# tonyzyl/ladcast

Measured on AMD Instinct MI355X. Metric: ensemble-member-steps/sec, higher is better.
Workload: dtype f32

## Files before the change

### include/ladcast_hip.h

```cpp
#ifndef LADCAST_HIP_H
#define LADCAST_HIP_H

#ifdef __cplusplus
extern "C" {
#endif

#define LDC_ABI_VERSION 5

#define LDC_OK 0
#define LDC_ERR_ARG (-1)
#define LDC_ERR_ALIGN (-2)
#define LDC_ERR_UNSUPPORTED (-3)

enum ldc_act { LDC_ACT_NONE = 0, LDC_ACT_SILU = 1, LDC_ACT_GELU_TANH = 2, LDC_ACT_RELU = 3 };
#define LDC_ACT_IN_TIMESTEP_SINCOS 16

int ldc_abi_version(void);
const char* ldc_build_arch(void);

typedef struct ldc_gemm_desc {
  int M, N, K, batch;
  int lda, ldw, ldc, ldr;
  long long a_bs, c_bs, r_bs;
  int gate_bs;
  int act;
  int flags;
  int reserved;
} ldc_gemm_desc;
#define LDC_GEMM_A_SPLIT 1
#define LDC_GEMM_C_SPLIT 2
#define LDC_GEMM_BF16_1TERM 4
#define LDC_GEMM_F32_REGSTAGE 8
#define LDC_FMT_F32 0
#define LDC_FMT_SPLIT 1
#define LDC_FMT_BF16 2
int ldc_sizeof_gemm_desc(void);
int ldc_gemm_bias_act(const float* A, const float* W, const float* bias, const float* gate,
                      const float* R, float* C, const ldc_gemm_desc* d, void* stream);

#define LDC_GEMM_MAX_PROBLEMS 4
typedef struct ldc_gemm_problem {
  const float* A;
  const float* W;
  const float* bias;
  const float* gate;
  const float* R;
  float* C;
  ldc_gemm_desc d;
} ldc_gemm_problem;
int ldc_sizeof_gemm_problem(void);
long long ldc_gemm_grouped_workspace_bytes(void);
int ldc_gemm_grouped_workspace_init(void* workspace, long long workspace_bytes, void* stream);
int ldc_gemm_grouped(const ldc_gemm_problem* problems, int n, void* workspace, long long workspace_bytes,
                     void* stream);

int ldc_gemm_grouped_bf16x3(const ldc_gemm_problem* problems, int n, void* workspace, long long workspace_bytes,
                            void* stream);
int ldc_pack_weight_bf16x2(const float* W, void* out, int N, int K, int ldw, void* stream);
int ldc_pack_weight_bf16(const float* W, void* out, int N, int K, int ldw, void* stream);

int ldc_linear_small(const float* x, int x_rows, const float* W, const float* bias,
                     const float* add, int add_rows, float* y, int rows, int N, int K,
                     int act_in, int act_out, void* stream);

int ldc_linear_small_mod(const float* x, int x_rows, const float* W, const float* bias, const float* add, int add_rows,
                         const float* mod, int mod_rows, float* y, int rows, int N, int K, int act_in, int act_out,
                         void* stream);

#define LDC_LINEAR_SMALL_MAX_GROUPED 4
typedef struct ldc_linear_small_problem {
  const float* x;
  const float* W;
  const float* bias;
  const float* add;
  float* y;
  int x_rows, add_rows, rows, N, K, act_in, act_out, reserved;
} ldc_linear_small_problem;
int ldc_linear_small_grouped(const ldc_linear_small_problem* problems, int n, void* stream);

int ldc_attn_fwd(const float* Q, const float* K, const float* V, float* O, int B, int S, int H,
                 int ld_qkv, long long qkv_bs, int ldo, long long o_bs, const float* key_bias, void* stream);
long long ldc_attn_fwd_workspace_bytes(void);
int ldc_attn_fwd_ws(const float* Q, const float* K, const float* V, float* O, int B, int S, int H, int ld_qkv, long long qkv_bs,
                    int ldo, long long o_bs, const float* key_bias, void* workspace, long long workspace_bytes, void* stream);
int ldc_attn_fwd_qrows(const float* Q, const float* K, const float* V, float* O, int B, int S, int Sq, int H, int ld_qkv,
                       long long qkv_bs, int ldo, long long o_bs, const float* key_bias, void* stream);
int ldc_attn_fwd_ws_qrows(const float* Q, const float* K, const float* V, float* O, int B, int S, int Sq, int H, int ld_qkv,
// ... 237 lines not shown
```

### ladcast_amd/csrc/gemm_bf16x3_v3.hip

```cpp
#include <math.h>
#include <stdio.h>
#include <stdlib.h>

#include "common.h"

namespace {

#include "gemm_v3_common.inc"
#include "gemm_v3_kstep_f32.inc"

struct SKArgs {
  DevProblem pr[MAXP];
  int np;
  int G;
  long long U;
  long long tiles;
  float* ws;
  unsigned* counters;
  unsigned upg, urem;
};

__device__ __forceinline__ long long range_start(long long g, const SKArgs& a) {
  const unsigned gu = static_cast<unsigned>(g);
  return static_cast<long long>(gu * a.upg + (gu < a.urem ? gu : a.urem));
}

__device__ __forceinline__ int find_problem_by_unit(const SKArgs& a, long long u) {
  int pi = 0;
#pragma unroll
  for (int k = 1; k < MAXP; ++k)
    if (k < a.np && u >= a.pr[k].unit0) pi = k;
  return pi;
}

#ifdef LDC_GEMM_STAMPS
#define LDC_STAMP(i)                                                                                        \
  if (threadIdx.x == 0)                                                                                     \
    reinterpret_cast<unsigned long long*>(a.counters)[65536 + blockIdx.x * 16 + (i)] = __builtin_amdgcn_s_memrealtime();
#define LDC_STAMP_CLK(i)                                                                                    \
  if (threadIdx.x == 0)                                                                                     \
    reinterpret_cast<unsigned long long*>(a.counters)[65536 + blockIdx.x * 16 + (i)] = __builtin_amdgcn_s_memtime();
#else
#define LDC_STAMP(i)
#define LDC_STAMP_CLK(i)
#endif

template <int BM, int TERMS, bool CONV = false>
__global__ __launch_bounds__(512) void gemm_bf16x3_v3_kernel(SKArgs a) {
  constexpr int CPK = TERMS == 1 ? 2 * BK : BK;
  constexpr int RT = BM / 128;
  constexpr int NACC = RT * 8;
  constexpr int STAGE_B = (BM + BN) * ROW_B;
  constexpr int SLOT_FLOATS = BM * BN;
  constexpr int NAI = BM / 64;
  constexpr int ND = NAI + 2;
  constexpr int NDH = ND / 2;
  extern __shared__ __attribute__((aligned(16))) unsigned char smem[];
  const int wave = __builtin_amdgcn_readfirstlane(static_cast<int>(threadIdx.x) >> 6);
  LDC_STAMP(0)
  int seg_ = 0;
  (void)seg_;
  int g;
  {
    const int bid = blockIdx.x, G = a.G;
    const int q = G >> 3, r = G & 7, xcd = bid & 7;
    g = (xcd < r ? xcd * (q + 1) : r * (q + 1) + (xcd - r) * q) + (bid >> 3);
  }
  auto uniform64 = [](long long v) {
    const unsigned lo = __builtin_amdgcn_readfirstlane(static_cast<unsigned>(v));
    const unsigned hi = __builtin_amdgcn_readfirstlane(static_cast<unsigned>(static_cast<unsigned long long>(v) >> 32));
    return static_cast<long long>((static_cast<unsigned long long>(hi) << 32) | lo);
  };
  const long long u_begin = uniform64(range_start(g, a));
  const long long u_end = uniform64(range_start(g + 1, a));
  const unsigned smem_lds = lds_addr(smem);

  struct Seg {
    int pi, tile, k0, k1, b, bm, bn;
  };
  auto decode = [&](long long u_) {
    Seg sg;
    sg.pi = find_problem_by_unit(a, u_);
    const DevProblem& Q = a.pr[sg.pi];
    const unsigned local = static_cast<unsigned>(u_ - Q.unit0), kt_u = static_cast<unsigned>(Q.kt);
    sg.tile = __builtin_amdgcn_readfirstlane(static_cast<int>(local / kt_u));
    sg.k0 = static_cast<int>(local - static_cast<unsigned>(sg.tile) * kt_u);
    const long long left = u_end - u_;
    sg.k1 = (Q.kt - sg.k0 <= left) ? Q.kt : sg.k0 + static_cast<int>(left);
    const unsigned per_b = static_cast<unsigned>(Q.tm * Q.tn), tile_u = static_cast<unsigned>(sg.tile);
    const unsigned b_ = tile_u / per_b;
    const unsigned t_in = tile_u - b_ * per_b;
    const unsigned strip = static_cast<unsigned>(Q.rm * Q.tn);
    const unsigned sr = t_in / strip;
    const unsigned r_in = t_in - sr * strip;
    const int rest = Q.tm - static_cast<int>(sr) * Q.rm;
    const unsigned h_sr = static_cast<unsigned>(rest < Q.rm ? rest : Q.rm);
    const unsigned bn_ = r_in / h_sr;
    sg.b = __builtin_amdgcn_readfirstlane(static_cast<int>(b_));
    sg.bn = __builtin_amdgcn_readfirstlane(static_cast<int>(bn_));
    sg.bm = __builtin_amdgcn_readfirstlane(static_cast<int>(sr) * Q.rm + static_cast<int>(r_in - bn_ * h_sr));
    return sg;
  };
  auto prefetch_next = [&](const Seg& sg) __attribute__((always_inline)) {
    const DevProblem& Q = a.pr[sg.pi];
    const int ln = fresh_lane();
    const int lr_ = ln >> 3, lp_ = ln & 7;
    const float* __restrict__ An = Q.A + static_cast<long long>(sg.b) * Q.d.a_bs;
    const long long wrb = static_cast<long long>(Q.d.K) * (TERMS == 1 ? 2 : 4);
    unsigned char* dump = smem + NSTAGE * STAGE_B + wave * 1024;
#pragma unroll
    for (int j = 0; j < 2; ++j) {
      const bool live = sg.k0 + j < sg.k1;
      const long long koff = static_cast<long long>(live ? sg.k0 + j : sg.k1 - 1) * (BK * 4);
      unsigned char* sA = smem + j * STAGE_B;
      unsigned char* sW = sA + BM * ROW_B;
#pragma unroll
      for (int i = 0; i < NAI; ++i) {
        const int r = 8 * (wave + 8 * i) + lr_;
        int gm = sg.bm * BM + r;
        gm = gm < Q.d.M ? gm : Q.d.M - 1;
        dma16(reinterpret_cast<const unsigned char*>(An + static_cast<long long>(gm) * Q.d.lda) + ((lp_ ^ swz(r)) << 4) + koff,
              live ? sA + (wave + 8 * i) * 1024 : dump);
      }
#pragma unroll
      for (int i = 0; i < 2; ++i) {
        const int r = 8 * (wave + 8 * i) + lr_;
        int gn = sg.bn * BN + r;
        gn = gn < Q.d.N ? gn : Q.d.N - 1;
        dma16(Q.W + static_cast<long long>(gn) * wrb + ((lp_ ^ swz(r)) << 4) + koff, live ? sW + (wave + 8 * (i)) * 1024 : dump);
      }
    }
  };
  long long u = u_begin;
// ... 304 lines not shown
#undef LDC_MMF
#undef LDC_MM
#undef LDC_RD_A
#undef LDC_RD_W
#undef LDC_SB
    __builtin_amdgcn_s_barrier();
    prefetched = false;
    if constexpr (!CONV && TERMS == 0) {
#if !defined(LDC_GEMM_DIAG_NODMA) && !defined(LDC_GEMM_NO_PREFETCH)
      if (u_next < u_end) {
        prefetch_next(nxt);
        prefetched = true;
      }
#endif
    }
    if (seg_ == 0) { LDC_STAMP_CLK(14) }
    LDC_STAMP(2 + 4 * seg_)

    if (k0 == 0 && k1 == P.kt) {
      tile_epilogue<BM, !CONV, LinearRows<BM>, true, TERMS == 0>(P, b, bm, bn, acc, wave, lane);
    } else {
      const int lane_h = fresh_lane();
      float* slot = a.ws + (static_cast<long long>(2 * g) + (k0 > 0 ? 0 : 1)) * SLOT_FLOATS + lane_h;
#pragma unroll
      for (int i = 0; i < NACC; ++i)
#pragma unroll
        for (int r = 0; r < 4; ++r)
          __hip_atomic_store(slot + ((wave * NACC + i) * 4 + r) * 64, acc[i][r], __ATOMIC_RELAXED, __HIP_MEMORY_SCOPE_AGENT);
      asm volatile("s_waitcnt vmcnt(0)" ::: "memory");
      __builtin_amdgcn_s_barrier();
      const long long f = P.unit0 + static_cast<long long>(tile) * P.kt;
      const long long l = f + P.kt;
      long long g_first = g;
      while (g_first > 0 && range_start(g_first, a) > f) --g_first;
      long long g_last = g;
      while (g_last + 1 < a.G && range_start(g_last + 1, a) < l) ++g_last;
      const unsigned pieces = static_cast<unsigned>(g_last - g_first + 1);
      unsigned* cnt = a.counters + (P.tile0 + tile);
      unsigned* flag = reinterpret_cast<unsigned*>(smem + NSTAGE * STAGE_B);
      if (wave == 0 && lane_h == 0) {
        const unsigned ticket = __hip_atomic_fetch_add(cnt, 1u, __ATOMIC_RELAXED, __HIP_MEMORY_SCOPE_AGENT);
        const unsigned last = (ticket == pieces - 1) ? 1u : 0u;
        if (last) {
          __builtin_amdgcn_fence(__ATOMIC_ACQUIRE, "agent");
          asm volatile("s_waitcnt vmcnt(0)" ::: "memory");
          __hip_atomic_store(cnt, 0u, __ATOMIC_RELAXED, __HIP_MEMORY_SCOPE_AGENT);
        }
        *flag = last;
      }
      __syncthreads();
      LDC_STAMP(3 + 4 * seg_)
      const unsigned is_last = *flag;
      __syncthreads();
      if (is_last) {
#pragma unroll
        for (int i = 0; i < NACC; ++i) acc[i] = f32x4{0.f, 0.f, 0.f, 0.f};
        for (long long gp = g_first; gp <= g_last; ++gp) {
          const long long s = range_start(gp, a);
          const float* sl = a.ws + (2 * gp + (s > f ? 0 : 1)) * SLOT_FLOATS;
#pragma unroll
          for (int i = 0; i < NACC; ++i) {
#pragma unroll
            for (int r = 0; r < 4; ++r) acc[i][r] += sl[((wave * NACC + i) * 4 + r) * 64 + lane_h];
          }
        }
        tile_epilogue<BM, !CONV, LinearRows<BM>, true, TERMS == 0>(P, b, bm, bn, acc, wave, lane);
      }
    }
    u = u_next;
    cur = nxt;
    LDC_STAMP(4 + 4 * seg_)
#ifdef LDC_GEMM_STAMPS
    if (seg_ < 2) ++seg_;
#endif
  }
  LDC_STAMP(15)
}

struct ConvParams {
  int H, W, cin, ks, kshift;
};

constexpr int LDC_SPLIT_GROUP = -100;

template <int BM, int TERMS, bool CONV = false>
int launch_v3(const ldc_gemm_problem* problems, const ldc_qkv_epilogue* epi, int n, void* workspace, long long workspace_bytes,
              void* stream, const ConvParams* cp = nullptr, bool may_split_group = false) {
  constexpr int SLOT_FLOATS = BM * BN;
  constexpr int STAGE_B = (BM + BN) * ROW_B;
  constexpr int CUS = 256;
  SKArgs a{};
  a.np = n;
  long long U = 0, tiles = 0;
  for (int i = 0; i < n; ++i) {
    const ldc_gemm_problem& q = problems[i];
    LDC_CHECK_PTR(q.A);
    LDC_CHECK_PTR(q.W);
    LDC_CHECK_PTR(q.C);
    const ldc_gemm_desc& d = q.d;
    if (d.M <= 0 || d.N <= 0 || d.K <= 0 || d.batch <= 0) return LDC_ERR_ARG;
    if (d.K % (TERMS == 1 ? 2 * BK : BK)) return LDC_ERR_UNSUPPORTED;
    if constexpr (TERMS == 0) {
      if (d.flags != 0 || d.ldw != d.K) return LDC_ERR_UNSUPPORTED;
    } else {
      if (!(d.flags & LDC_GEMM_A_SPLIT)) return LDC_ERR_UNSUPPORTED;
    }
    LDC_CHECK_ALIGN16(q.A);
    LDC_CHECK_ALIGN16(q.W);
    if constexpr (TERMS == 0) {
      if ((d.lda & 3) || (d.a_bs & 3)) return LDC_ERR_UNSUPPORTED;
    } else {
      if ((d.lda & 7) || (d.a_bs & 7) || (reinterpret_cast<unsigned long long>(q.A) & 31ull)) return LDC_ERR_ALIGN;
    }
    if (d.act < LDC_ACT_NONE || d.act > LDC_ACT_RELU) return LDC_ERR_UNSUPPORTED;
    DevProblem& P = a.pr[i];
    P.A = q.A;
    P.W = reinterpret_cast<const unsigned char*>(q.W);
    P.bias = q.bias;
    P.gate = q.gate;
    P.R = q.R;
// ... 105 lines not shown
  }
  if constexpr (TERMS == 0) {
    if (U >= 4 * CUS) G = CUS;
  }
  static const char* const force_g = LDC_AB_GETENV("LDC_BF16X3_G");
  if (force_g) {
    const long long g_ = atoll(force_g);
    if (g_ > 0 && g_ <= CUS) G = g_;
  }
  if (U < G) G = U;
  if (workspace == nullptr) return LDC_ERR_ARG;
  if (workspace_bytes < LDC_GEMM_COUNTER_BYTES + 2 * slot_bytes) return LDC_ERR_ARG;
  {
    const long long fit = (workspace_bytes - LDC_GEMM_COUNTER_BYTES) / (2 * slot_bytes);
    if (fit < G) G = fit;
  }
  LDC_CHECK_ALIGN16(workspace);
  if (U >= (1LL << 31)) return LDC_ERR_UNSUPPORTED;
#ifdef LDC_AB_BUILD
  {
    static const bool dbg = getenv("LDC_GEMM_DEBUG_G") != nullptr;
    if (dbg)
      fprintf(stderr, "ldc_gemm cut: terms %d conv %d n %d tiles %lld kt0 %d BM %d G %lld U %lld %s\n", TERMS, int(CONV), n, tiles, a.pr[0].kt, BM, G, U,
              (U % G == 0 && (U / G) % a.pr[0].kt == 0) ? "whole tiles" : (U % G == 0 ? "equal ranges" : "UNALIGNED"));
  }
#endif
  a.G = static_cast<int>(G);
  a.U = U;
  a.upg = static_cast<unsigned>(U / G);
  a.urem = static_cast<unsigned>(U % G);
  a.tiles = tiles;
  a.ws = reinterpret_cast<float*>(static_cast<unsigned char*>(workspace) + LDC_GEMM_COUNTER_BYTES);
  a.counters = static_cast<unsigned*>(workspace);
  const size_t lds = NSTAGE * STAGE_B + 8 * 1024;
  static const bool attr_set = [&] {
    (void)hipFuncSetAttribute(reinterpret_cast<const void*>(gemm_bf16x3_v3_kernel<BM, TERMS, CONV>),
                              hipFuncAttributeMaxDynamicSharedMemorySize, static_cast<int>(lds));
    return true;
  }();
  (void)attr_set;
  hipLaunchKernelGGL((gemm_bf16x3_v3_kernel<BM, TERMS, CONV>), dim3(a.G), dim3(512), lds, static_cast<hipStream_t>(stream), a);
  return ldc_launch_status();
}

}

static int gemm_v3_dispatch(const ldc_gemm_problem* problems, const ldc_qkv_epilogue* epi, int n, void* workspace,
                            long long workspace_bytes, void* stream) {
  LDC_CHECK_PTR(problems);
  if (n <= 0 || n > MAXP) return LDC_ERR_ARG;
  long long tiles256 = 0;
  for (int i = 0; i < n; ++i) {
    const ldc_gemm_desc& d = problems[i].d;
    if (d.M <= 0 || d.N <= 0 || d.batch <= 0) return LDC_ERR_ARG;
    if (!(d.flags & LDC_GEMM_A_SPLIT)) return LDC_ERR_UNSUPPORTED;
    if (((d.flags ^ problems[0].d.flags) & LDC_GEMM_BF16_1TERM) != 0) return LDC_ERR_ARG;
    tiles256 += static_cast<long long>(d.batch) * ldc_cdiv(d.M, 256) * ldc_cdiv(d.N, BN);
  }
  static const char* const force_thr = LDC_AB_GETENV("LDC_BF16X3_SMALL_TILES");
  bool small = tiles256 < (force_thr ? atoll(force_thr) : 400);
  static const char* const force_bm = LDC_AB_GETENV("LDC_BF16X3_BM");
  if (force_bm) small = (atoi(force_bm) == 128);
  const bool one = (problems[0].d.flags & LDC_GEMM_BF16_1TERM) != 0;
  auto launch = [&](const ldc_gemm_problem* pr, const ldc_qkv_epilogue* ep, int cnt, bool sm, bool may_split) {
    if (one)
      return sm ? launch_v3<128, 1>(pr, ep, cnt, workspace, workspace_bytes, stream, nullptr, may_split)
                : launch_v3<256, 1>(pr, ep, cnt, workspace, workspace_bytes, stream, nullptr, may_split);
    return sm ? launch_v3<128, 3>(pr, ep, cnt, workspace, workspace_bytes, stream, nullptr, may_split)
              : launch_v3<256, 3>(pr, ep, cnt, workspace, workspace_bytes, stream, nullptr, may_split);
  };
  const int st = launch(problems, epi, n, small, true);
  if (st != LDC_SPLIT_GROUP) return st;
  for (int i = 0; i < n; ++i) {
    const ldc_gemm_desc& d = problems[i].d;
    bool sm = static_cast<long long>(d.batch) * ldc_cdiv(d.M, 256) * ldc_cdiv(d.N, BN) < (force_thr ? atoll(force_thr) : 400);
    if (force_bm) sm = (atoi(force_bm) == 128);
    const int sti = launch(problems + i, epi ? epi + i : nullptr, 1, sm, false);
    if (sti != LDC_OK) return sti;
  }
  return LDC_OK;
}

static int gemm_f32_ring(const ldc_gemm_problem* problems, const ldc_qkv_epilogue* epi, int n, void* workspace, long long workspace_bytes,
                         void* stream) {
  LDC_CHECK_PTR(problems);
  if (n <= 0 || n > MAXP) return LDC_ERR_ARG;
  for (int i = 0; i < n; ++i)
    if (problems[i].d.flags & LDC_GEMM_F32_REGSTAGE) return LDC_ERR_UNSUPPORTED;
  auto al16 = [](const void* q_) { return q_ != nullptr && (reinterpret_cast<unsigned long long>(q_) & 15ull) == 0; };
  if (!al16(workspace) || workspace_bytes < LDC_GEMM_COUNTER_BYTES + 2ll * 256 * BN * static_cast<long long>(sizeof(float)))
    return LDC_ERR_UNSUPPORTED;
  for (int i = 0; i < n; ++i) {
    const ldc_gemm_desc& d = problems[i].d;
    if (d.M <= 0 || d.N <= 0 || d.K <= 0 || d.batch <= 0) return LDC_ERR_ARG;
    if (!al16(problems[i].A) || !al16(problems[i].W)) return LDC_ERR_UNSUPPORTED;
  }
#ifdef LDC_AB_BUILD
  static const char* const force_bm = getenv("LDC_F32_RING_BM");
  if (force_bm && atoi(force_bm) == 256) return launch_v3<256, 0>(problems, epi, n, workspace, workspace_bytes, stream);
#endif
  return launch_v3<128, 0>(problems, epi, n, workspace, workspace_bytes, stream);
}

int ldc_gemm_grouped_f32_ring(const ldc_gemm_problem* problems, int n, void* workspace, long long workspace_bytes, void* stream) {
  return gemm_f32_ring(problems, nullptr, n, workspace, workspace_bytes, stream);
}

extern "C" int ldc_gemm_grouped_qkv_f32(const ldc_gemm_problem* problems, const ldc_qkv_epilogue* epi, int n, void* workspace,
                                        long long workspace_bytes, void* stream) {
  LDC_CHECK_PTR(epi);
  return gemm_f32_ring(problems, epi, n, workspace, workspace_bytes, stream);
}

int ldc_gemm_grouped_bf16x3_v3(const ldc_gemm_problem* problems, int n, void* workspace, long long workspace_bytes,
                               void* stream) {
  return gemm_v3_dispatch(problems, nullptr, n, workspace, workspace_bytes, stream);
}

extern "C" int ldc_gemm_grouped_bf16x3_qkv(const ldc_gemm_problem* problems, const ldc_qkv_epilogue* epi, int n, void* workspace,
                                           long long workspace_bytes, void* stream) {
  LDC_CHECK_PTR(epi);
  return gemm_v3_dispatch(problems, epi, n, workspace, workspace_bytes, stream);
}

extern "C" int ldc_sphere_conv_nhwc_split(const float* X, const void* Wp, const float* bias, const float* R, float* Y, int B, int H,
                                          int W, int cin, int ldx, int cout, int ldy, int ldr, int ksize, int act, int in_fmt,
                                          int out_fmt, void* workspace, long long workspace_bytes, void* stream) {
  LDC_CHECK_PTR(X);
  LDC_CHECK_PTR(Wp);
  LDC_CHECK_PTR(Y);
  if (B <= 0 || H <= 0 || W <= 0 || cin <= 0 || cout <= 0) return LDC_ERR_ARG;
  if (ksize != 1 && ksize != 3 && ksize != 5) return LDC_ERR_UNSUPPORTED;
  if (ksize > 1 && ((W & 1) || H < 2 || H < ksize / 2 || W / 2 < ksize / 2 || H > 32767 || W > 65535)) return LDC_ERR_UNSUPPORTED;
  if (in_fmt != LDC_FMT_SPLIT && in_fmt != LDC_FMT_BF16 && in_fmt != LDC_FMT_F32) return LDC_ERR_UNSUPPORTED;
// ... 52 lines not shown
```

### ladcast_amd/hip.py

```python
from __future__ import annotations

import ctypes
import os
from ctypes import POINTER, Structure, c_char_p, c_double, c_float, c_int, c_longlong, c_void_p

import torch

_HERE = os.path.dirname(os.path.abspath(__file__))
LIB_PATH = os.environ.get("LDC_LIB_PATH") or os.path.join(_HERE, "libladcast_hip.so")

ACT_NONE, ACT_SILU, ACT_GELU_TANH, ACT_RELU = 0, 1, 2, 3
ACT_IN_TIMESTEP_SINCOS = 16
GEMM_A_SPLIT, GEMM_C_SPLIT, GEMM_BF16_1TERM = 1, 2, 4
GEMM_F32_REGSTAGE = 8
ATTN_OUT_SPLIT, ATTN_BF16_1TERM, ATTN_OUT_BF16 = 1, 2, 4
ABI_VERSION = 5
FMT_F32, FMT_SPLIT, FMT_BF16 = 0, 1, 2


class GemmDesc(Structure):
    _fields_ = [
        ("M", c_int), ("N", c_int), ("K", c_int), ("batch", c_int),
        ("lda", c_int), ("ldw", c_int), ("ldc", c_int), ("ldr", c_int),
        ("a_bs", c_longlong), ("c_bs", c_longlong), ("r_bs", c_longlong),
        ("gate_bs", c_int), ("act", c_int), ("flags", c_int), ("reserved", c_int),
    ]


class GemmProblem(Structure):
    _fields_ = [("A", c_void_p), ("W", c_void_p), ("bias", c_void_p), ("gate", c_void_p), ("R", c_void_p), ("C", c_void_p), ("d", GemmDesc)]


MAX_GROUPED = 4


class QkvEpilogue(Structure):
    _fields_ = [("wq", c_void_p), ("wk", c_void_p), ("rope", c_void_p), ("reserved", c_void_p), ("eps", c_float), ("qscale", c_float),
                ("heads", c_int), ("rope_row0", c_int)]


class LinearSmallProblem(Structure):
    _fields_ = [("x", c_void_p), ("W", c_void_p), ("bias", c_void_p), ("add", c_void_p), ("y", c_void_p), ("x_rows", c_int), ("add_rows", c_int),
                ("rows", c_int), ("N", c_int), ("K", c_int), ("act_in", c_int), ("act_out", c_int), ("reserved", c_int)]


PRODUCTS_MAX_QUANTILES, PRODUCTS_MAX_THRESHOLDS, PRODUCTS_MAX_MEMBERS, PRODUCTS_MAX_SORT_MEMBERS = 16, 8, 1024, 64


class ProductsDesc(Structure):
    _fields_ = [("n_quant", c_int), ("n_thr", c_int), ("q_lo", c_int * PRODUCTS_MAX_QUANTILES), ("q_t", c_float * PRODUCTS_MAX_QUANTILES),
                ("thr_dir", c_int * PRODUCTS_MAX_THRESHOLDS)]


EVENTS_MAX, EVENTS_MAX_MEMBERS = 32, 1024


class EventsDesc(Structure):
    _fields_ = [("n_events", c_int), ("channel", c_int * EVENTS_MAX), ("dir", c_int * EVENTS_MAX), ("anomaly", c_int * EVENTS_MAX),
                ("thr", c_float * EVENTS_MAX)]


def _load():
    if not os.path.exists(LIB_PATH):
        raise RuntimeError(
            f"{LIB_PATH} is missing: build it with `python -c 'import __graft_entry__ as g; g.build()'` "
            "(or `make -C ladcast_amd/csrc`).  ladcast_amd has no CPU fallback."
        )
    lib = ctypes.CDLL(LIB_PATH)
    P, I, L, F, D = c_void_p, c_int, c_longlong, c_float, c_double
    sig = {
        "ldc_abi_version": (I, []),
        "ldc_build_arch": (c_char_p, []),
        "ldc_sizeof_gemm_desc": (I, []),
        "ldc_gemm_bias_act": (I, [P, P, P, P, P, P, POINTER(GemmDesc), P]),
        "ldc_sizeof_gemm_problem": (I, []),
        "ldc_gemm_grouped_workspace_bytes": (L, []),
        "ldc_gemm_grouped_workspace_init": (I, [P, L, P]),
        "ldc_gemm_grouped": (I, [POINTER(GemmProblem), I, P, L, P]),
        "ldc_gemm_grouped_bf16x3": (I, [POINTER(GemmProblem), I, P, L, P]),
        "ldc_sizeof_qkv_epilogue": (I, []),
        "ldc_gemm_grouped_bf16x3_qkv": (I, [POINTER(GemmProblem), POINTER(QkvEpilogue), I, P, L, P]),
        "ldc_gemm_grouped_qkv_f32": (I, [POINTER(GemmProblem), POINTER(QkvEpilogue), I, P, L, P]),
        "ldc_attn_qkv_prepare_split": (I, [P, P, P, I, I, I, I, L, I, P, P, P, P, P, P, P, P, F, P]),
        "ldc_attn_fwd_split_workspace_bytes": (L, [I, I, I]),
        "ldc_attn_fwd_split_workspace_max_bytes": (L, []),
        "ldc_attn_fwd_split": (I, [P, P, P, P, I, I, I, I, L, I, L, P, I, P, L, P]),
        "ldc_attn_fwd_split_qrows_workspace_bytes": (L, [I, I, I, I]),
        "ldc_attn_fwd_split_qrows": (I, [P, P, P, P, I, I, I, I, I, L, I, L, P, I, P, L, P]),
        "ldc_pack_weight_bf16x2": (I, [P, P, I, I, I, P]),
        "ldc_pack_weight_bf16": (I, [P, P, I, I, I, P]),
        "ldc_linear_small": (I, [P, I, P, P, P, I, P, I, I, I, I, I, P]),
        "ldc_linear_small_grouped": (I, [POINTER(LinearSmallProblem), I, P]),
        "ldc_linear_small_mod": (I, [P, I, P, P, P, I, P, I, P, I, I, I, I, I, P]),
        "ldc_gate_residual_layernorm": (I, [P, P, P, P, I, I, I, I, L, I, L, I, I, L, P, P, F, I, P]),
        "ldc_attn_fwd": (I, [P, P, P, P, I, I, I, I, L, I, L, P, P]),
        "ldc_attn_fwd_ws": (I, [P, P, P, P, I, I, I, I, L, I, L, P, P, L, P]),
        "ldc_attn_fwd_qrows": (I, [P, P, P, P, I, I, I, I, I, L, I, L, P, P]),
        "ldc_attn_fwd_ws_qrows": (I, [P, P, P, P, I, I, I, I, I, L, I, L, P, P, L, P]),
        "ldc_attn_fwd_ws_qrows_thr": (I, [P, P, P, P, I, I, I, I, I, L, I, L, P, P, L, F, P]),
        "ldc_attn_fwd_workspace_bytes": (L, []),
        "ldc_qk_rmsnorm_rope": (I, [P, P, I, I, I, I, I, L, P, P, F, P, P, P]),
        "ldc_sphere_conv_nhwc_split": (I, [P, P, P, P, P, I, I, I, I, I, I, I, I, I, I, I, I, P, L, P]),
        "ldc_sphere_conv_plan": (I, [I, I, I, I, I, I, I, P, P]),
        "ldc_rmsnorm_rows_split": (I, [P, P, P, P, P, P, L, I, I, I, I, I, I, F, I, P]),
        "ldc_pixel_unshuffle_shortcut_split": (I, [P, P, P, P, I, I, I, I, I, I, I, P]),
        "ldc_pixel_shuffle_shortcut_split": (I, [P, P, P, P, I, I, I, I, I, I, I, P]),
        "ldc_pixel_shuffle_to_chan": (I, [P, P, I, I, I, I, I, P]),
        "ldc_split_rows": (I, [P, P, L, I, I, I, I, P]),
        "ldc_upsample_nearest2x_rows": (I, [P, P, P, I, I, I, I, I, I, I, I, P]),
        "ldc_sphere_dwconv_nhwc_fmt": (I, [P, P, P, P, I, I, I, I, I, I, I, I, I, P]),
        "ldc_relu_linear_attn_nhwc_fmt": (I, [P, P, I, I, I, I, I, F, I, P, L, P]),
# ... 36 lines not shown
        "ldc_ddpm_step": (I, [P, P, P, P, P, F, F, F, F, F, F, I, L, P]),
        "ldc_scale_f32": (I, [P, F, P, L, P]),
        "ldc_axpby_f32": (I, [P, F, P, F, P, L, P]),
        "ldc_edm_noise_inputs": (I, [P, P, P, P, P, P, I, L, P]),
        "ldc_edm_denoise": (I, [P, P, P, P, P, I, I, I, I, I, I, I, P]),
        "ldc_edm_denoise_loss": (I, [P, P, P, P, P, P, P, P, P, I, I, I, I, I, P]),
        "ldc_sphere_conv_nhwc": (I, [P, P, P, P, P, I, I, I, I, I, I, I, I, I, I, P]),
        "ldc_sphere_dwconv_nhwc": (I, [P, P, P, P, I, I, I, I, I, I, I, I, P]),
        "ldc_grouped_conv1x1_nhwc": (I, [P, P, P, L, I, I, I, P]),
        "ldc_relu_linear_attn_nhwc": (I, [P, P, I, I, I, I, I, F, P, L, P]),
        "ldc_relu_linear_attn_workspace_bytes": (L, [I, I, I]),
        "ldc_rmsnorm_rows": (I, [P, P, P, P, P, L, I, I, I, I, F, I, P]),
        "ldc_pixel_unshuffle_shortcut": (I, [P, P, P, I, I, I, I, I, P]),
        "ldc_pixel_shuffle_shortcut": (I, [P, P, P, I, I, I, I, I, P]),
        "ldc_chan_regroup": (I, [P, P, L, I, I, P]),
        "ldc_track_gather": (I, [P, L, L, L, I, I, L, POINTER(c_int), I, P, P, F, P, I, I, P]),
        "ldc_track_nanmean": (I, [P, L, I, L, P, P]),
        "ldc_track_storms": (I, [P, L, L, L, L, P, P, I, P, I, P, P, I, I, POINTER(c_int), I, I, P, P, P, P]),
        "ldc_track_local_min": (I, [P, L, P, P, I, P, I, P, P, P, I, P, P, P, P, P]),
        "ldc_recon_preprocess": (I, [P, L, L, L, I, I, I, I, P, P, I, P, P, P]),
        "ldc_recon_scores_workspace_bytes": (L, [I, I, I, I]),
        "ldc_recon_scores": (I, [P, P, P, L, P, P, P, P, I, I, I, I, I, I, P, P, P, P, L, P]),
        "ldc_field_moments_workspace_bytes": (L, [I, I, I, I]),
        "ldc_field_moments": (I, [P, L, L, L, I, I, I, I, P, I, P, L, P]),
    }
    for name, (res, args) in sig.items():
        fn = getattr(lib, name)
        fn.restype = res
        fn.argtypes = args
    if lib.ldc_abi_version() != ABI_VERSION:
        raise RuntimeError("libladcast_hip.so ABI version mismatch")
    if lib.ldc_sizeof_gemm_desc() != ctypes.sizeof(GemmDesc) or lib.ldc_sizeof_gemm_problem() != ctypes.sizeof(GemmProblem):
        raise RuntimeError("ldc_gemm_desc / ldc_gemm_problem layout mismatch between header and binding")
    if lib.ldc_sizeof_qkv_epilogue() != ctypes.sizeof(QkvEpilogue):
        raise RuntimeError("ldc_qkv_epilogue layout mismatch between header and binding")
    if lib.ldc_sizeof_products_desc() != ctypes.sizeof(ProductsDesc):
        raise RuntimeError("ldc_products_desc layout mismatch between header and binding")
    if lib.ldc_sizeof_events_desc() != ctypes.sizeof(EventsDesc):
        raise RuntimeError("ldc_events_desc layout mismatch between header and binding")
    return lib, sig


lib, SIGNATURES = _load()


def _check(status: int, what: str):
    if status != 0:
        raise RuntimeError(f"{what} failed with status {status}")


def upload_nonblocking(t, device):
    device = torch.device(device)
    if device.type != "cuda" or t.device.type != "cpu":
        return t.to(device)
    return (t if t.is_pinned() else t.pin_memory()).to(device, non_blocking=True)


def _p(t):
    return None if t is None else c_void_p(t.data_ptr())


def _stream():
    return c_void_p(torch.cuda.current_stream().cuda_stream)


def _dev(*ts):
# ... 22 lines not shown
            raise RuntimeError(f"{name}: the first call on a stream must be made outside a graph capture (run one warm-up forward)")
        if ws is not None:
            _outgrown.append(ws)
        ws = torch.empty((nbytes + 3) // 4, device=device, dtype=torch.float32)
        if init == "zero":
            ws.zero_()
        elif init == "grouped":
            _check(lib.ldc_gemm_grouped_workspace_init(c_void_p(ws.data_ptr()), ws.numel() * 4, _stream()), "ldc_gemm_grouped_workspace_init")
        _workspaces[key] = ws
    return ws


def _grouped_workspace(device):
    return _workspace("gemm_grouped", device, lib.ldc_gemm_grouped_workspace_bytes(), init="grouped")


def gemm_problem(A, W, C, *, M, N, K, batch=1, lda=None, ldw=None, ldc=None, a_bs=0, c_bs=0, bias=None, gate=None, gate_bs=0, R=None,
                 ldr=0, r_bs=0, act=ACT_NONE, flags=0):
    _dev(A, W, C, bias, gate, R)
    d = GemmDesc(M, N, K, batch, lda if lda is not None else K, ldw if ldw is not None else K, ldc if ldc is not None else N, ldr,
                 a_bs, c_bs, r_bs, gate_bs, act, flags, 0)
    pv = lambda t: None if t is None else t.data_ptr()
    return GemmProblem(pv(A), pv(W), pv(bias), pv(gate), pv(R), pv(C), d), (A, W, C, bias, gate, R)


def gemm_grouped(problems, split_bf16=False):
    n = len(problems)
    if not 1 <= n <= MAX_GROUPED:
        raise ValueError(f"gemm_grouped takes 1..{MAX_GROUPED} problems")
    arr = (GemmProblem * n)(*[p[0] for p in problems])
    ws = _grouped_workspace(problems[0][1][2].device)
    fn = lib.ldc_gemm_grouped_bf16x3 if split_bf16 else lib.ldc_gemm_grouped
    _check(fn(arr, n, c_void_p(ws.data_ptr()), ws.numel() * 4, _stream()), "ldc_gemm_grouped" + ("_bf16x3" if split_bf16 else ""))


def gemm_sk(A, W, C, split_bf16=False, **kw):
    gemm_grouped([gemm_problem(A, W, C, **kw)], split_bf16=split_bf16)


def pack_weight_bf16x2(W):
    _dev(W)
    W = W.contiguous()
    N, K = W.shape
    out = torch.empty(N * K, device=W.device, dtype=torch.int32)
    _check(lib.ldc_pack_weight_bf16x2(_p(W), _p(out), N, K, K, _stream()), "ldc_pack_weight_bf16x2")
    return out


def pack_weight_bf16(W):
    _dev(W)
    W = W.contiguous()
    N, K = W.shape
    out = torch.empty(N * K, device=W.device, dtype=torch.bfloat16)
    _check(lib.ldc_pack_weight_bf16(_p(W), _p(out), N, K, K, _stream()), "ldc_pack_weight_bf16")
    return out


def linear_small(x, W, y, *, rows, N, K, x_rows=None, bias=None, add=None, add_rows=1, act_in=ACT_NONE, act_out=ACT_NONE, mod=None, mod_rows=1):
    _dev(x, W, y, bias, add, mod)
    xr = x_rows if x_rows is not None else rows
    if mod is not None:
        _check(lib.ldc_linear_small_mod(_p(x), xr, _p(W), _p(bias), _p(add), add_rows, _p(mod), mod_rows, _p(y), rows, N, K, act_in, act_out, _stream()),
               "ldc_linear_small_mod")
        return
    _check(lib.ldc_linear_small(_p(x), xr, _p(W), _p(bias), _p(add), add_rows, _p(y), rows, N, K, act_in, act_out, _stream()), "ldc_linear_small")

# ... 629 lines not shown
```

Baseline: 3.255.

## Balance stream-K f32 GEMM unit ranges by cost to discount ragged edge tiles

Adds a host-side planner that assigns stream-K unit ranges per CU in proportion to estimated cost, treating the ragged last row-tile (few rows) as cheaper than full tiles. The start offsets are passed in a per-launch table inside the kernel arguments, replacing the uniform split for the f32 BM=128 path. The aim is to reduce load imbalance when partial-M tiles finish faster than full ones. In exchange the kernel argument struct grows by about 1 KiB, and the plan is recomputed on the host on every launch. A plan-query API and Python binding are also added.

```diff
diff --git a/include/ladcast_hip.h b/include/ladcast_hip.h
--- a/include/ladcast_hip.h
+++ b/include/ladcast_hip.h
@@ -53,6 +53,18 @@
 int ldc_gemm_grouped_workspace_init(void* workspace, long long workspace_bytes, void* stream);
 int ldc_gemm_grouped(const ldc_gemm_problem* problems, int n, void* workspace, long long workspace_bytes,
                      void* stream);
+
+#define LDC_GEMM_F32_PLAN_MAX_RANGES 256
+typedef struct ldc_gemm_f32_plan_t {
+  int G, by_cost, max_pieces, reserved;
+  long long units;
+  unsigned start[LDC_GEMM_F32_PLAN_MAX_RANGES + 1];
+  int ragged_tile[LDC_GEMM_MAX_PROBLEMS], ragged_rows[LDC_GEMM_MAX_PROBLEMS], unit_cost[LDC_GEMM_MAX_PROBLEMS], body[LDC_GEMM_MAX_PROBLEMS];
+  int kt[LDC_GEMM_MAX_PROBLEMS], tm[LDC_GEMM_MAX_PROBLEMS], tn[LDC_GEMM_MAX_PROBLEMS], rm[LDC_GEMM_MAX_PROBLEMS];
+  long long unit0[LDC_GEMM_MAX_PROBLEMS];
+} ldc_gemm_f32_plan_t;
+int ldc_sizeof_gemm_f32_plan(void);
+int ldc_gemm_f32_plan(const ldc_gemm_problem* problems, int n, long long workspace_bytes, ldc_gemm_f32_plan_t* plan);
 
 int ldc_gemm_grouped_bf16x3(const ldc_gemm_problem* problems, int n, void* workspace, long long workspace_bytes,
                             void* stream);
diff --git a/ladcast_amd/csrc/gemm_bf16x3_v3.hip b/ladcast_amd/csrc/gemm_bf16x3_v3.hip
--- a/ladcast_amd/csrc/gemm_bf16x3_v3.hip
+++ b/ladcast_amd/csrc/gemm_bf16x3_v3.hip
@@ -8,6 +8,8 @@
 
 #include "gemm_v3_common.inc"
 #include "gemm_v3_kstep_f32.inc"
+
+constexpr int MAX_RANGES = 256;
 
 struct SKArgs {
   DevProblem pr[MAXP];
@@ -18,11 +20,31 @@
   float* ws;
   unsigned* counters;
   unsigned upg, urem;
+  unsigned start[MAX_RANGES + 1];
 };
-
+static_assert(sizeof(SKArgs) <= 4096, "SKArgs travels by value in the kernarg segment (4 KiB)");
+
+template <bool TABLE>
 __device__ __forceinline__ long long range_start(long long g, const SKArgs& a) {
   const unsigned gu = static_cast<unsigned>(g);
+  if constexpr (TABLE) return static_cast<long long>(a.start[gu]);
   return static_cast<long long>(gu * a.upg + (gu < a.urem ? gu : a.urem));
+}
+
+struct TileCoord {
+  int b, bm, bn;
+};
+__host__ __device__ __forceinline__ TileCoord tile_coord(int tm, int tn, int rm, unsigned tile_u) {
+  const unsigned per_b = static_cast<unsigned>(tm * tn);
+  const unsigned b_ = tile_u / per_b;
+  const unsigned t_in = tile_u - b_ * per_b;
+  const unsigned strip = static_cast<unsigned>(rm * tn);
+  const unsigned sr = t_in / strip;
+  const unsigned r_in = t_in - sr * strip;
+  const int rest = tm - static_cast<int>(sr) * rm;
+  const unsigned h_sr = static_cast<unsigned>(rest < rm ? rest : rm);
+  const unsigned bn_ = r_in / h_sr;
+  return TileCoord{static_cast<int>(b_), static_cast<int>(sr) * rm + static_cast<int>(r_in - bn_ * h_sr), static_cast<int>(bn_)};
 }
 
 __device__ __forceinline__ int find_problem_by_unit(const SKArgs& a, long long u) {
@@ -49,6 +71,7 @@
 __global__ __launch_bounds__(512) void gemm_bf16x3_v3_kernel(SKArgs a) {
   constexpr int CPK = TERMS == 1 ? 2 * BK : BK;
   constexpr int RT = BM / 128;
+  constexpr bool TABLE = BM == 128 && TERMS == 0 && !CONV;
   constexpr int NACC = RT * 8;
   constexpr int STAGE_B = (BM + BN) * ROW_B;
   constexpr int SLOT_FLOATS = BM * BN;
@@ -71,8 +94,8 @@
     const unsigned hi = __builtin_amdgcn_readfirstlane(static_cast<unsigned>(static_cast<unsigned long long>(v) >> 32));
     return static_cast<long long>((static_cast<unsigned long long>(hi) << 32) | lo);
   };
-  const long long u_begin = uniform64(range_start(g, a));
-  const long long u_end = uniform64(range_start(g + 1, a));
+  const long long u_begin = uniform64(range_start<TABLE>(g, a));
+  const long long u_end = uniform64(range_start<TABLE>(g + 1, a));
   const unsigned smem_lds = lds_addr(smem);
 
   struct Seg {
@@ -87,18 +110,10 @@
     sg.k0 = static_cast<int>(local - static_cast<unsigned>(sg.tile) * kt_u);
     const long long left = u_end - u_;
     sg.k1 = (Q.kt - sg.k0 <= left) ? Q.kt : sg.k0 + static_cast<int>(left);
-    const unsigned per_b = static_cast<unsigned>(Q.tm * Q.tn), tile_u = static_cast<unsigned>(sg.tile);
-    const unsigned b_ = tile_u / per_b;
-    const unsigned t_in = tile_u - b_ * per_b;
-    const unsigned strip = static_cast<unsigned>(Q.rm * Q.tn);
-    const unsigned sr = t_in / strip;
-    const unsigned r_in = t_in - sr * strip;
-    const int rest = Q.tm - static_cast<int>(sr) * Q.rm;
-    const unsigned h_sr = static_cast<unsigned>(rest < Q.rm ? rest : Q.rm);
-    const unsigned bn_ = r_in / h_sr;
-    sg.b = __builtin_amdgcn_readfirstlane(static_cast<int>(b_));
-    sg.bn = __builtin_amdgcn_readfirstlane(static_cast<int>(bn_));
-    sg.bm = __builtin_amdgcn_readfirstlane(static_cast<int>(sr) * Q.rm + static_cast<int>(r_in - bn_ * h_sr));
+    const TileCoord tc = tile_coord(Q.tm, Q.tn, Q.rm, static_cast<unsigned>(sg.tile));
+    sg.b = __builtin_amdgcn_readfirstlane(tc.b);
+    sg.bn = __builtin_amdgcn_readfirstlane(tc.bn);
+    sg.bm = __builtin_amdgcn_readfirstlane(tc.bm);
     return sg;
   };
   auto prefetch_next = [&](const Seg& sg) __attribute__((always_inline)) {
@@ -469,9 +484,9 @@
       const long long f = P.unit0 + static_cast<long long>(tile) * P.kt;
       const long long l = f + P.kt;
       long long g_first = g;
-      while (g_first > 0 && range_start(g_first, a) > f) --g_first;
+      while (g_first > 0 && range_start<TABLE>(g_first, a) > f) --g_first;
       long long g_last = g;
-      while (g_last + 1 < a.G && range_start(g_last + 1, a) < l) ++g_last;
+      while (g_last + 1 < a.G && range_start<TABLE>(g_last + 1, a) < l) ++g_last;
       const unsigned pieces = static_cast<unsigned>(g_last - g_first + 1);
       unsigned* cnt = a.counters + (P.tile0 + tile);
       unsigned* flag = reinterpret_cast<unsigned*>(smem + NSTAGE * STAGE_B);
@@ -493,7 +508,7 @@
 #pragma unroll
         for (int i = 0; i < NACC; ++i) acc[i] = f32x4{0.f, 0.f, 0.f, 0.f};
         for (long long gp = g_first; gp <= g_last; ++gp) {
-          const long long s = range_start(gp, a);
+          const long long s = range_start<TABLE>(gp, a);
           const float* sl = a.ws + (2 * gp + (s > f ? 0 : 1)) * SLOT_FLOATS;
 #pragma unroll
           for (int i = 0; i < NACC; ++i) {
@@ -514,6 +529,86 @@
   LDC_STAMP(15)
 }
 
+constexpr int UNIT_COST_WHOLE = 8;
+inline int ragged_unit_cost(int rows) {
+  int low = 5;
+  if (const char* e = LDC_AB_GETENV("LDC_GEMM_F32_RAGGED_COST")) low = atoi(e);
+  return (rows + 15) / 16 <= 4 && low >= 1 && low <= UNIT_COST_WHOLE ? low : UNIT_COST_WHOLE;
+}
+
+struct RangePlan {
+  int by_cost;
+  int max_pieces;
+  int ragged_rows[MAXP];
+  int ragged_cost[MAXP];
+};
+
+inline int max_pieces_per_tile(const SKArgs& a, const unsigned* s) {
+  int worst = 1, g = 0;
+  for (int pi = 0; pi < a.np; ++pi) {
+    const DevProblem& P = a.pr[pi];
+    const long long nt = static_cast<long long>(P.d.batch) * P.tm * P.tn;
+    for (long long t = 0; t < nt; ++t) {
+      const long long f = P.unit0 + t * P.kt, l = f + P.kt;
+      while (static_cast<long long>(s[g + 1]) <= f) ++g;
+      int ge = g;
+      while (static_cast<long long>(s[ge + 1]) < l) ++ge;
+      if (ge - g + 1 > worst) worst = ge - g + 1;
+    }
+  }
+  return worst;
+}
+
+inline RangePlan plan_ranges(SKArgs& a) {
+  RangePlan rp{};
+  const int G = a.G;
+  const long long U = a.U;
+  for (unsigned g = 0; g <= static_cast<unsigned>(G); ++g) a.start[g] = g * a.upg + (g < a.urem ? g : a.urem);
+  long long C = 0;
+  bool cheap = false;
+  for (int pi = 0; pi < a.np; ++pi) {
+    const DevProblem& P = a.pr[pi];
+    const int rows = P.d.M - (P.tm - 1) * 128;
+    const int c = rows < 128 ? ragged_unit_cost(rows) : UNIT_COST_WHOLE;
+    rp.ragged_cost[pi] = c;
+    rp.ragged_rows[pi] = c < UNIT_COST_WHOLE ? rows : 0;
+    cheap = cheap || c < UNIT_COST_WHOLE;
+    const long long nt = static_cast<long long>(P.d.batch) * P.tm * P.tn, nr = static_cast<long long>(P.d.batch) * P.tn;
+    C += ((nt - nr) * UNIT_COST_WHOLE + nr * c) * P.kt;
+  }
+  rp.max_pieces = max_pieces_per_tile(a, a.start);
+  if (!cheap || U < 4 * MAX_RANGES || G < 2) return rp;
+  unsigned s[MAX_RANGES + 1];
+  const long long cpg = C / G, crem = C % G;
+  auto target = [&](long long g) { return g * cpg + (g < crem ? g : crem); };
+  long long S = 0;
+  int g = 1;
+  s[0] = 0;
+  for (int pi = 0; pi < a.np && g < G; ++pi) {
+    const DevProblem& P = a.pr[pi];
+    const long long nt = static_cast<long long>(P.d.batch) * P.tm * P.tn;
+    for (long long t = 0; t < nt && g < G; ++t) {
+      const int c = tile_coord(P.tm, P.tn, P.rm, static_cast<unsigned>(t)).bm == P.tm - 1 ? rp.ragged_cost[pi] : UNIT_COST_WHOLE;
+      const long long tile_cost = static_cast<long long>(c) * P.kt;
+      while (g < G && target(g) <= S + tile_cost) {
+        s[g] = static_cast<unsigned>(P.unit0 + t * P.kt + (target(g) - S + c - 1) / c);
+        ++g;
+      }
+      S += tile_cost;
+    }
+  }
+  if (g != G) return rp;
+  s[G] = static_cast<unsigned>(U);
+  for (int i = 0; i < G; ++i)
+    if (s[i] >= s[i + 1]) return rp;
+  const int pieces = max_pieces_per_tile(a, s);
+  if (pieces > rp.max_pieces) return rp;
+  for (int i = 0; i <= G; ++i) a.start[i] = s[i];
+  rp.by_cost = 1;
+  rp.max_pieces = pieces;
+  return rp;
+}
+
 struct ConvParams {
   int H, W, cin, ks, kshift;
 };
@@ -522,7 +617,7 @@
 
 template <int BM, int TERMS, bool CONV = false>
 int launch_v3(const ldc_gemm_problem* problems, const ldc_qkv_epilogue* epi, int n, void* workspace, long long workspace_bytes,
-              void* stream, const ConvParams* cp = nullptr, bool may_split_group = false) {
+              void* stream, const ConvParams* cp = nullptr, bool may_split_group = false, ldc_gemm_f32_plan_t* plan = nullptr) {
   constexpr int SLOT_FLOATS = BM * BN;
   constexpr int STAGE_B = (BM + BN) * ROW_B;
   constexpr int CUS = 256;
@@ -694,6 +789,30 @@
   a.tiles = tiles;
   a.ws = reinterpret_cast<float*>(static_cast<unsigned char*>(workspace) + LDC_GEMM_COUNTER_BYTES);
   a.counters = static_cast<unsigned*>(workspace);
+  if constexpr (BM == 128 && TERMS == 0 && !CONV) {
+    static_assert(CUS == MAX_RANGES, "SKArgs::start holds one entry per CU");
+    const RangePlan rp = plan_ranges(a);
+    if (plan != nullptr) {
+      plan->G = a.G;
+      plan->by_cost = rp.by_cost;
+      plan->max_pieces = rp.max_pieces;
+      plan->units = U;
+      for (int g = 0; g <= a.G; ++g) plan->start[g] = a.start[g];
+      for (int i = 0; i < n; ++i) {
+        plan->ragged_tile[i] = rp.ragged_rows[i] ? a.pr[i].tm - 1 : -1;
+        plan->ragged_rows[i] = rp.ragged_rows[i];
+        plan->unit_cost[i] = rp.ragged_cost[i];
+        plan->body[i] = 0;
+        plan->unit0[i] = a.pr[i].unit0;
+        plan->kt[i] = a.pr[i].kt;
+        plan->tm[i] = a.pr[i].tm;
+        plan->tn[i] = a.pr[i].tn;
+        plan->rm[i] = a.pr[i].rm;
+      }
+      return LDC_OK;
+    }
+  }
+  if (plan != nullptr) return LDC_ERR_UNSUPPORTED;
   const size_t lds = NSTAGE * STAGE_B + 8 * 1024;
   static const bool attr_set = [&] {
     (void)hipFuncSetAttribute(reinterpret_cast<const void*>(gemm_bf16x3_v3_kernel<BM, TERMS, CONV>),
@@ -744,7 +863,7 @@
 }
 
 static int gemm_f32_ring(const ldc_gemm_problem* problems, const ldc_qkv_epilogue* epi, int n, void* workspace, long long workspace_bytes,
-                         void* stream) {
+                         void* stream, ldc_gemm_f32_plan_t* plan = nullptr) {
   LDC_CHECK_PTR(problems);
   if (n <= 0 || n > MAXP) return LDC_ERR_ARG;
   for (int i = 0; i < n; ++i)
@@ -761,7 +880,16 @@
   static const char* const force_bm = getenv("LDC_F32_RING_BM");
   if (force_bm && atoi(force_bm) == 256) return launch_v3<256, 0>(problems, epi, n, workspace, workspace_bytes, stream);
 #endif
-  return launch_v3<128, 0>(problems, epi, n, workspace, workspace_bytes, stream);
+  return launch_v3<128, 0>(problems, epi, n, workspace, workspace_bytes, stream, nullptr, false, plan);
+}
+
+static_assert(LDC_GEMM_F32_PLAN_MAX_RANGES == MAX_RANGES, "ldc_gemm_f32_plan_t::start holds one entry per unit range");
+extern "C" int ldc_sizeof_gemm_f32_plan(void) { return static_cast<int>(sizeof(ldc_gemm_f32_plan_t)); }
+extern "C" int ldc_gemm_f32_plan(const ldc_gemm_problem* problems, int n, long long workspace_bytes, ldc_gemm_f32_plan_t* plan) {
+  LDC_CHECK_PTR(plan);
+  *plan = ldc_gemm_f32_plan_t{};
+  return gemm_f32_ring(problems, nullptr, n, reinterpret_cast<void*>(static_cast<unsigned long long>(LDC_GEMM_COUNTER_BYTES)), workspace_bytes, nullptr,
+                       plan);
 }
 
 int ldc_gemm_grouped_f32_ring(const ldc_gemm_problem* problems, int n, void* workspace, long long workspace_bytes, void* stream) {
diff --git a/ladcast_amd/hip.py b/ladcast_amd/hip.py
--- a/ladcast_amd/hip.py
+++ b/ladcast_amd/hip.py
@@ -2,7 +2,7 @@
 
 import ctypes
 import os
-from ctypes import POINTER, Structure, c_char_p, c_double, c_float, c_int, c_longlong, c_void_p
+from ctypes import POINTER, Structure, c_char_p, c_double, c_float, c_int, c_longlong, c_uint, c_void_p
 
 import torch
 
@@ -32,6 +32,15 @@
 
 
 MAX_GROUPED = 4
+GEMM_F32_PLAN_MAX_RANGES = 256
+
+
+class GemmF32Plan(Structure):
+    _fields_ = [("G", c_int), ("by_cost", c_int), ("max_pieces", c_int), ("reserved", c_int), ("units", c_longlong),
+                ("start", c_uint * (GEMM_F32_PLAN_MAX_RANGES + 1)),
+                ("ragged_tile", c_int * MAX_GROUPED), ("ragged_rows", c_int * MAX_GROUPED), ("unit_cost", c_int * MAX_GROUPED), ("body", c_int * MAX_GROUPED),
+                ("kt", c_int * MAX_GROUPED), ("tm", c_int * MAX_GROUPED), ("tn", c_int * MAX_GROUPED), ("rm", c_int * MAX_GROUPED),
+                ("unit0", c_longlong * MAX_GROUPED)]
 
 
 class QkvEpilogue(Structure):
@@ -77,6 +86,8 @@
         "ldc_gemm_grouped_workspace_bytes": (L, []),
         "ldc_gemm_grouped_workspace_init": (I, [P, L, P]),
         "ldc_gemm_grouped": (I, [POINTER(GemmProblem), I, P, L, P]),
+        "ldc_sizeof_gemm_f32_plan": (I, []),
+        "ldc_gemm_f32_plan": (I, [POINTER(GemmProblem), I, L, POINTER(GemmF32Plan)]),
         "ldc_gemm_grouped_bf16x3": (I, [POINTER(GemmProblem), I, P, L, P]),
         "ldc_sizeof_qkv_epilogue": (I, []),
         "ldc_gemm_grouped_bf16x3_qkv": (I, [POINTER(GemmProblem), POINTER(QkvEpilogue), I, P, L, P]),
@@ -179,6 +190,8 @@
         raise RuntimeError("libladcast_hip.so ABI version mismatch")
     if lib.ldc_sizeof_gemm_desc() != ctypes.sizeof(GemmDesc) or lib.ldc_sizeof_gemm_problem() != ctypes.sizeof(GemmProblem):
         raise RuntimeError("ldc_gemm_desc / ldc_gemm_problem layout mismatch between header and binding")
+    if lib.ldc_sizeof_gemm_f32_plan() != ctypes.sizeof(GemmF32Plan):
+        raise RuntimeError("ldc_gemm_f32_plan_t layout mismatch between header and binding")
     if lib.ldc_sizeof_qkv_epilogue() != ctypes.sizeof(QkvEpilogue):
         raise RuntimeError("ldc_qkv_epilogue layout mismatch between header and binding")
     if lib.ldc_sizeof_products_desc() != ctypes.sizeof(ProductsDesc):
@@ -267,6 +280,24 @@
     ws = _grouped_workspace(problems[0][1][2].device)
     fn = lib.ldc_gemm_grouped_bf16x3 if split_bf16 else lib.ldc_gemm_grouped
     _check(fn(arr, n, c_void_p(ws.data_ptr()), ws.numel() * 4, _stream()), "ldc_gemm_grouped" + ("_bf16x3" if split_bf16 else ""))
+
+
+def gemm_f32_plan(shapes, workspace_bytes=None):
+    n = len(shapes)
+    if not 1 <= n <= MAX_GROUPED:
+        raise ValueError(f"gemm_f32_plan takes 1..{MAX_GROUPED} problems")
+    arr = (GemmProblem * n)()
+    for q, sh in zip(arr, shapes):
+        M, N, K = sh[:3]
+        batch = sh[3] if len(sh) > 3 else 1
+        q.A = q.W = q.C = 4096
+        q.d = GemmDesc(M, N, K, batch, K, K, N, 0, M * K, M * N, 0, 0, ACT_NONE, 0, 0)
+    plan = GemmF32Plan()
+    nbytes = int(lib.ldc_gemm_grouped_workspace_bytes()) if workspace_bytes is None else int(workspace_bytes)
+    _check(lib.ldc_gemm_f32_plan(arr, n, nbytes, ctypes.byref(plan)), "ldc_gemm_f32_plan")
+    per = lambda f: [int(v) for v in getattr(plan, f)[:n]]
+    return dict(G=plan.G, start=[int(v) for v in plan.start[: plan.G + 1]], by_cost=bool(plan.by_cost), max_pieces=plan.max_pieces, units=int(plan.units),
+                **{f: per(f) for f in ("ragged_tile", "ragged_rows", "unit_cost", "body", "unit0", "kt", "tm", "tn", "rm")})
 
 
 def gemm_sk(A, W, C, split_bf16=False, **kw):
```

Result: no change. 3.281, median of 6 (+0.8%).
